# gunrock/mini

Measured on AMD Instinct MI355X. Metric: MTEPS (million traversed edges/sec) BFS advance+filter, RMAT-22, higher is better.
Workload: dtype int32

## Files before the change

### include/mgx/bfs_fused.hpp

```cpp
#pragma once
#include <cstdlib>
#include <cstring>

#include "runtime.hpp"
#include "env.hpp"
#include "wave.hpp"

namespace mgx {

constexpr int BFS_MAX_TRACE = 4096;
constexpr int BFS_VSHIFT = 38;
constexpr u64 BFS_EMASK = (1ull << BFS_VSHIFT) - 1ull;

struct bfs_ctrl_t {
  u64 cursor[3];
  u64 pad_a_[13];
  u64 lcursor[3];
  u64 pad_b_[13];
  u64 ledges[3];
  u64 pad_c_[13];
  u64 reached;
  u64 pad_d_[15];
  u64 merged_new;
  u64 sum_edges;
  u64 sum_frontier;
  u64 sum_long_edges;
  u64 sum_long_vertices;
  u64 claims;
  u64 claims_level[64];
  u64 pull_edges;
  int done;
  int levels;
  int pull;
  int push_levels;
  int d2_append_level;
// ... 173 lines not shown
  c->vshort_slots = 0;
  c->lazy_slot = -1;
  c->lazy_slots = 0;
  c->cold_slot = -1;
  c->cold_slots = 0;
  c->mini_slots = 0;
  for (int i = 0; i < 4; ++i) c->mini_blocks[i] = 0u;
  c->reached_mini = 0;
  c->d2_frozen_level = -1;
  for (int i = 0; i < 16; ++i) ((u32*)c->d2_level_kind)[i] = 0u;
  for (int i = 0; i < 64; ++i) c->d2_level_new[i] = 0u;
  c->sssp_thr = 0x7f7fffffu;
  c->sssp_far_cnt[0] = c->sssp_far_cnt[1] = 0;
  c->sssp_far_min[0] = c->sssp_far_min[1] = 0x7f7fffffu;
  for (int i = 0; i < 64; ++i) c->stamp[i] = 0;
}

__host__ __device__ __forceinline__ u32 bfs_lq_pad(u32 deg) { return (deg + 63u) & ~63u; }
__host__ __device__ __forceinline__ u32 bfs_lq_degree(u32 entry, u32 next_entry) {
  return ((next_entry & ~63u) - (entry & ~63u)) - ((64u - (entry & 63u)) & 63u);
}

__device__ __forceinline__ void bfs_seed_queue(const bfs_fused_args_t& a, u32 row) {
  bfs_ctrl_t* c = a.ctrl;
  const u32 ro = a.row_offsets[row];
  const u32 deg = a.row_offsets[row + 1] - ro;
  const bool is_long = a.long_min > 0 && deg >= (u32)a.long_min;
  (is_long ? a.lq_row : a.fr_row)[0][0] = ro;
  (is_long ? a.lq_off : a.fr_off)[0][0] = is_long ? (deg & 63u) : 0u;
  (is_long ? c->lcursor : c->cursor)[0] = deg ? ((1ull << BFS_VSHIFT) | (u64)(is_long ? bfs_lq_pad(deg) : deg)) : 0ull;
  if (is_long) c->ledges[0] = deg;
}

__global__ __launch_bounds__(BLOCK) void k_bfs_fused_init(bfs_fused_args_t a, int src, long long nwords, const bfs_ctrl_t* prev_ctrl,
                                                          bfs_ctrl_t* prev_head, int head_words) {
  if (prev_head && blockIdx.x == 0) {
    const u32* const from = (const u32*)prev_ctrl;
    u32* const to = (u32*)prev_head;
    for (int i = threadIdx.x; i < head_words; i += BLOCK) to[i] = from[i];
    __syncthreads();
  }
  const int src_old = src;
  if (a.new_of_old) src = a.new_of_old[src];
  const long long tid = (long long)blockIdx.x * BLOCK + threadIdx.x;
  const long long nth = (long long)gridDim.x * BLOCK;
  const long long n = a.n;
  for (long long i = tid; i < (n + 3) / 4; i += nth) {
    if (i * 4 + 4 <= n) {
      const long long j = i * 4;
      const int4 l = make_int4(src_old == j ? 0 : -1, src_old == j + 1 ? 0 : -1, src_old == j + 2 ? 0 : -1,
                               src_old == j + 3 ? 0 : -1);
      *(int4*)(a.labels + j) = l;
      *(u32*)(a.mark + i * 4) = 0u;
    } else {
      for (long long j = i * 4; j < n; ++j) { a.labels[j] = (j == src_old) ? 0 : -1; a.mark[j] = 0; }
    }
  }
  const u32 src_bit = 1u << (src & 31);
  for (long long w = tid; w < nwords; w += nth) {
    const u32 seed = (w == (src >> 5)) ? src_bit : 0u;
    a.visited[w] = seed;
    a.frontier_bits[w] = seed;
  }
  if (tid == 0) {
    bfs_ctrl_reset(a.ctrl);
    bfs_slot_marks_clear(a, 0);
    bfs_slot_marks_clear(a, 1);
    bfs_seed_queue(a, (u32)src);
  }
}

__device__ __forceinline__ bool bfs_open_level(const bfs_fused_args_t& a, int level, int slot) {
  bfs_ctrl_t* const c = a.ctrl;
  const u64 cur = c->cursor[slot % 3];
  const u64 lcur = c->lcursor[slot % 3];
  const long long nf = (long long)(cur >> BFS_VSHIFT) + (long long)(lcur >> BFS_VSHIFT);
  const u64 long_edges = c->ledges[slot % 3];
  const u64 E = (cur & BFS_EMASK) + long_edges;
  c->cursor[(slot + 2) % 3] = 0;
  c->lcursor[(slot + 2) % 3] = 0;
  c->ledges[(slot + 2) % 3] = 0;
  if (level < 64) c->stamp[level] = __builtin_amdgcn_s_memrealtime();
  if (nf == 0) {
    if (!c->done) { c->done = 1; c->levels = level; }
    return false;
  }
  if (level < BFS_MAX_TRACE) c->trace[level] = ((u64)nf << BFS_VSHIFT) | E;
  c->sum_edges += E;
  c->sum_frontier += (u64)nf;
  c->sum_long_edges += long_edges;
  c->sum_long_vertices += lcur >> BFS_VSHIFT;
  if (a.mode == 1 && !c->pull) {
    const float unvisited = (float)((long long)a.n - (long long)c->reached);
    if (unvisited < (float)nf * a.alpha) c->pull = 1;
  }
  if (!c->pull) c->push_levels += 1;
  return true;
}

__device__ __forceinline__ bool bfs_level_pulls(const bfs_fused_args_t& a, const bfs_ctrl_t* c, int slot) {
  if (a.mode != 1) return false;
  if (c->pull) return true;
// ... 542 lines not shown
  u32* __restrict__ const out_row_s = a.fr_row[(slot + 1) & 1];
  u32* __restrict__ const out_off_s = a.fr_off[(slot + 1) & 1];
  u32* __restrict__ const out_row_l = a.lq_row[(slot + 1) & 1];
  u32* __restrict__ const out_off_l = a.lq_off[(slot + 1) & 1];
  const u64 base_s = s_base[0], base_l = s_base[1];
#pragma unroll
  for (int q = 0; q < 16; ++q) {
    if ((new16 >> q) & 1u) {
      const u32 deg = ro[q + 1] - ro[q];
      if (deg >= long_min) {
        const u64 at = (base_l >> BFS_VSHIFT) + (ex_l >> 40);
        out_row_l[at] = ro[q];
        out_off_l[at] = (u32)((base_l & BFS_EMASK) + (ex_l & DEGMASK)) | (deg & 63u);
        ex_l += CNT1 | (u64)bfs_lq_pad(deg);
      } else if (deg) {
        const u64 at = (base_s >> BFS_VSHIFT) + (ex_s >> 40);
        out_row_s[at] = ro[q];
        out_off_s[at] = (u32)((base_s & BFS_EMASK) + (ex_s & DEGMASK));
        ex_s += CNT1 | (u64)deg;
      }
    }
  }
}

__global__ void k_bfs_publish(const bfs_ctrl_t* __restrict__ c, bfs_ctrl_t* __restrict__ host, u64* host_seq, u64 seq, int words) {
  const u32* const src = (const u32*)c;
  u32* const dst = (u32*)host;
  for (int i = threadIdx.x; i < words; i += blockDim.x) dst[i] = src[i];
  __threadfence_system();
  __syncthreads();
  if (threadIdx.x == 0) __hip_atomic_store(host_seq, seq, __ATOMIC_RELEASE, __HIP_MEMORY_SCOPE_SYSTEM);
}

struct bfs_run_opts_t {
  int cold_test = -1;
  int merged = 1;
  int dense = -1;
  int vshort = -1;
  long long chain = -1;
  int pack24 = 1;
  int hot_units = 1;
  int cold_pack = 1;
  int src_plan = 1;
  int defer_words = -1;
  int defer_mul = 1, defer_div = 1;
  int do_chain = 1;
  int merged_pull = 1;
  int seed_chain = 1;
  int tail_chain = 1;
  int tail_front = 1;
  int chain_big = -1;
  int cold = 1;
  int lazy = -1;
  long long defer = -1;
  int spin = -1;
  int build_list = 0;
  int mini = 1;
  int many_spare = 0;
#ifdef MGX_LAB
  int flags = 0;
  int build_diag = 0;
  int dense_diag = 0;
#endif
  static bfs_run_opts_t from_env() {
    bfs_run_opts_t o;
    auto geti = [](const char* name, int& out) { if (const char* e = mgx::env(name)) out = atoi(e); };
    auto getll = [](const char* name, long long& out) { if (const char* e = mgx::env(name)) out = atoll(e); };
    geti("MGX_BFS_COLD_TEST", o.cold_test);
    geti("MGX_BFS_MERGED_PUSH", o.merged);
    geti("MGX_BFS_DENSE", o.dense);
    geti("MGX_BFS_VSHORT", o.vshort);
    getll("MGX_BFS_CHAIN_MAX_EDGES", o.chain);
    geti("MGX_BFS_BUILD_LIST", o.build_list);
    getll("MGX_BFS_DEFER", o.defer);
    geti("MGX_BFS_DEFER_WORDS", o.defer_words);
    geti("MGX_BFS_SRC_PLAN", o.src_plan);
    geti("MGX_BFS_PACK24", o.pack24);
    geti("MGX_BFS_COLD_PACK", o.cold_pack);
    geti("MGX_BFS_HOT_UNITS", o.hot_units);
    geti("MGX_BFS_COLD", o.cold);
    if (const char* e = mgx::env("MGX_BFS_DEFER_REACH")) {
      o.defer_mul = atoi(e);
      const char* sl = strchr(e, '/');
      o.defer_div = sl ? atoi(sl + 1) : 1;
      if (o.defer_div < 1) o.defer_div = 1;
    }
    geti("MGX_BFS_SEED_CHAIN", o.seed_chain);
    geti("MGX_BFS_MERGED_PULL", o.merged_pull);
    geti("MGX_BFS_DO_CHAIN", o.do_chain);
    geti("MGX_BFS_TAIL_CHAIN", o.tail_chain);
    geti("MGX_BFS_TAIL_FRONT", o.tail_front);
    geti("MGX_BFS_CHAIN_BIG_EDGES", o.chain_big);
    geti("MGX_BFS_MINI", o.mini);
    if (o.many_spare < 0) o.many_spare = 0;
    geti("MGX_BFS_LAZY", o.lazy);
    if (o.lazy > (1 << 20)) o.lazy = 1 << 20;
#ifdef MGX_LAB
    geti("MGX_BFS_FLAGS", o.flags);
    geti("MGX_BFS_BUILD_DIAG", o.build_diag);
    geti("MGX_BFS_DENSE_DIAG", o.dense_diag);
#else
#endif
    return o;
  }
};

struct bfs_fused_state_t {
  bfs_run_opts_t opts = bfs_run_opts_t::from_env();
  mem_t<u32> visited;
  mem_t<unsigned char> mark;
  mem_t<u32> frontier_bits;
  mem_t<u32> fr_row[2];
  mem_t<u32> fr_off[2];
  mem_t<u32> lq_row[2];
  mem_t<u32> lq_off[2];
  mem_t<bfs_ctrl_t> ctrl;
  mem_t<u32> flush_buf;
  unsigned defer_min_marks = 2048;
  bfs_ctrl_t* host_ctrl = nullptr;
  u64* host_seq = nullptr;
  u64 seq = 0;
  bool spin = true;
  int n = 0;
  int levels_per_sync = 2;
  int slots_hint = 5;
  int slots_used = 0;
  bool time_batches = false;
  unsigned chain_max_edges = 4096;
  unsigned vshort_div = 8;
  unsigned chain_big_edges = 4096;
  int recent_need[4] = {1, 1, 1, 1}, recent_at = 0;
  int cls_max[3] = {0, 0, 0}, cls_at[3] = {0, 0, 0};
  int auto_spare = 0, clean_batches = 0;
  int tail_from = 1 << 30;
  unsigned lazy_div = 4;
  mem_t<u32> slot_marks;
  mem_t<u32> cold_flush;
  unsigned dense_div = 2;
  int long_min = LONG_MIN_DEFAULT;
  bool count_marks = false;
  int time_kernels = 0;
  unsigned hot_min_edges = 65536;
  hipEvent_t ev0 = nullptr, ev1 = nullptr;
  double level_kernel_ms = 0.0;
  long long level_kernel_launches = 0;
  float batch_ms[256];
  int batches = 0;
  static constexpr int EV_POOL = 96;
  hipEvent_t wev[EV_POOL] = {};
  double wave_kernel_ms = 0.0;
  long long wave_kernel_launches = 0;
  double stream_kernel_ms = 0.0;
  long long stream_kernel_launches = 0;
  float level_stream_ms[64] = {};
  float level_wave_ms[64] = {};

  bfs_fused_state_t(int num_nodes, standard_context_t& ctx) : n(num_nodes) {
    size_t words = (size_t)(num_nodes + 31) / 32 + 8;
    if (words < 65536) words = 65536;
    visited = mem_t<u32>(words, ctx);
    frontier_bits = mem_t<u32>(words, ctx);
    mark = mem_t<unsigned char>((size_t)num_nodes + 64, ctx);
    MGX_HIP(hipMemsetAsync(visited.data(), 0, words * sizeof(u32), ctx.stream()));
    MGX_HIP(hipMemsetAsync(frontier_bits.data(), 0, words * sizeof(u32), ctx.stream()));
    for (int i = 0; i < 2; ++i) {
      fr_row[i] = mem_t<u32>((size_t)num_nodes + 1, ctx);
      fr_off[i] = mem_t<u32>((size_t)num_nodes + 1, ctx);
      lq_row[i] = mem_t<u32>((size_t)num_nodes + 1, ctx);
      lq_off[i] = mem_t<u32>((size_t)num_nodes + 1, ctx);
    }
// ... 24 lines not shown
```

### include/mgx/bfs_fused_mini.hpp

```cpp
#pragma once
#include "bfs_fused.hpp"
#include "bfs_fused_chain.hpp"

namespace mgx {

constexpr int BFS_MINI_WGS = 64;
constexpr int BFS_MINI_LCAP = 4096;
constexpr int BFS_MINI_WCAP = 8192;
constexpr u32 BFS_MINI_EDGES_LATE = 131072;
constexpr u32 BFS_MINI_EDGES_EARLY = 32768;
constexpr u32 BFS_MINI_SHORT_ROWS = 65536;
constexpr size_t bfs_mini_lds_bytes() {
  return (size_t)(2 * BFS_MINI_LCAP + 4) * 4 + (size_t)BFS_MINI_WCAP * 4 + 64 * 8 + 256;
}

__device__ __forceinline__ bool bfs_level_is_mini(const bfs_fused_args_t& a, const bfs_ctrl_t* c, int slot) {
  if (a.mode != 0 || c->lazy_slot == slot) return false;
  const u64 cur = c->cursor[slot % 3], lcur = c->lcursor[slot % 3];
  const u64 E = (cur & BFS_EMASK) + c->ledges[slot % 3];
  const bool late = c->reached * 4ull >= (u64)(u32)a.n;
  return (lcur >> BFS_VSHIFT) <= (u64)BFS_MINI_LCAP && (cur >> BFS_VSHIFT) <= (u64)BFS_MINI_SHORT_ROWS &&
         E <= (u64)(late ? BFS_MINI_EDGES_LATE : BFS_MINI_EDGES_EARLY);
}

template <int NT>
__global__ __launch_bounds__(NT) void k_bfs_mini(bfs_fused_args_t a, int arg) {
  constexpr int NW = NT / WAVE;
  constexpr u64 CNT1 = 1ull << 40;
  constexpr u64 DEGMASK = CNT1 - 1ull;
  extern __shared__ __attribute__((aligned(16))) char smem[];
  u32* const s_loff = (u32*)smem;
  u32* const s_lrow = s_loff + BFS_MINI_LCAP + 4;
  u32* const s_win = s_lrow + BFS_MINI_LCAP;
  u64* const s_scan = (u64*)(s_win + BFS_MINI_WCAP);
  __shared__ int s_cnt, s_maxdeg;
  __shared__ u64 s_base[2];
  __shared__ u32 s_long_true;
  bfs_ctrl_t* const c = a.ctrl;
  int slot, level;
  bfs_resolve(c, arg, slot, level);
  if (c->done) return;
  const u64 cur = c->cursor[slot % 3], lcur = c->lcursor[slot % 3];
  const u64 ledges = c->ledges[slot % 3];
  const int nf_s = (int)(cur >> BFS_VSHIFT), nf_l = (int)(lcur >> BFS_VSHIFT);
  const u32 Es = (u32)(cur & BFS_EMASK), Rl = (u32)(lcur & BFS_EMASK);
  const int in = slot & 1, out = (slot + 1) & 1;
  const bool first_thread = blockIdx.x == 0 && threadIdx.x == 0;
  if (nf_s + nf_l == 0) {
    if (first_thread) {
      c->cursor[(slot + 2) % 3] = 0; c->lcursor[(slot + 2) % 3] = 0; c->ledges[(slot + 2) % 3] = 0;
      if (level < 64) c->stamp[level] = __builtin_amdgcn_s_memrealtime();
      if (!c->done) { c->done = 1; c->levels = level; }
    }
    return;
  }
  const long long gtid = (long long)blockIdx.x * NT + threadIdx.x, gthreads = (long long)gridDim.x * NT;
  if (!bfs_level_is_mini(a, c, slot)) {
    const bool lazy = c->lazy_slot == slot;
    const bool fb = c->fb_slot == slot;
    if (!lazy) {
      for (long long i = gtid; i < nf_s; i += gthreads) { a.fr_row[out][i] = a.fr_row[in][i]; a.fr_off[out][i] = a.fr_off[in][i]; }
      for (long long i = gtid; i < nf_l; i += gthreads) { a.lq_row[out][i] = a.lq_row[in][i]; a.lq_off[out][i] = a.lq_off[in][i]; }
    }
    __syncthreads();
    if (threadIdx.x == 0) {
      __threadfence();
      if (atomicAdd(&c->mini_blocks[slot & 3], 1u) == gridDim.x - 1u) {
        c->mini_blocks[slot & 3] = 0u;
        c->cursor[(slot + 1) % 3] = cur; c->lcursor[(slot + 1) % 3] = lcur; c->ledges[(slot + 1) % 3] = ledges;
        c->cursor[(slot + 2) % 3] = 0; c->lcursor[(slot + 2) % 3] = 0; c->ledges[(slot + 2) % 3] = 0;
        c->slot_level[(slot + 1) & 3] = level;
        c->flush_count[(slot + 1) & 1] = 0;
        bfs_slot_marks_clear(a, slot + 1);
        if (lazy) c->lazy_slot = slot + 1;
        if (fb) c->fb_slot = slot + 1;
      }
    }
    return;
  }
  if (first_thread) {
    const u64 E = (u64)Es + ledges;
    c->cursor[(slot + 2) % 3] = 0; c->lcursor[(slot + 2) % 3] = 0; c->ledges[(slot + 2) % 3] = 0;
    if (level < 64) c->stamp[level] = __builtin_amdgcn_s_memrealtime();
    if (level < BFS_MAX_TRACE) c->trace[level] = ((u64)(nf_s + nf_l) << BFS_VSHIFT) | E;
    c->sum_edges += E;
    c->sum_frontier += (u64)(nf_s + nf_l);
    c->sum_long_edges += ledges;
    c->sum_long_vertices += (u64)nf_l;
    c->push_levels += 1;
    c->small_levels += 1;
    c->mini_slots += 1;
    c->slots += 1;
    c->slot_level[(slot + 1) & 3] = level + 1;
    c->flush_count[(slot + 1) & 1] = 0;
    bfs_slot_marks_clear(a, slot + 1);
    c->fb_slot = -1;
  }
  const int lane = lane_id();
  const int wave = threadIdx.x / WAVE;
  const u32 long_min = a.long_min > 0 ? (u32)a.long_min : 0xFFFFFFFFu;
// ... 38 lines not shown
        if (tot_l >> 40) atomicAdd(&c->ledges[(slot + 1) % 3], (u64)s_long_true);
      }
      __syncthreads();
      if (deg) {
        const u64 b = is_long ? s_base[1] : s_base[0];
        const u64 at = is_long ? ex_l : ex_s;
        const u64 pos = (b >> BFS_VSHIFT) + (at >> 40);
        (is_long ? out_row_l : out_row_s)[pos] = ro;
        (is_long ? out_off_l : out_off_s)[pos] = (u32)((b & BFS_EMASK) + (at & DEGMASK)) | (is_long ? (deg & 63u) : 0u);
      }
      __syncthreads();
    }
    if (threadIdx.x == 0) s_cnt = 0;
    __syncthreads();
  };
  auto visit = [&](bool act, u32 d) {
    bool win = false;
    if (act) {
      const u32 bit = 1u << (d & 31u);
      const u32 seen = a.visited[d >> 5];
      if (!(seen & bit)) win = !(atomicOr(a.visited + (d >> 5), bit) & bit);
    }
    const u64 bal = __ballot(win);
    if (bal) {
      int at = 0;
      if (lane == 0) at = atomicAdd(&s_cnt, __popcll(bal));
      at = __builtin_amdgcn_readfirstlane(at);
      if (win) { s_win[at + rank_in_mask(bal)] = d; ++found; }
    }
  };

  {
    const u32 U = Rl >> 6;
    const u32 Wt = (u32)gridDim.x * NW, w0 = (u32)blockIdx.x * NW + (u32)wave;
    const u32 iters = (U + Wt - 1u) / Wt;
    for (u32 t = 0; t < iters; ++t) {
      const u32 u = w0 + t * Wt;
      bool act = false;
      u32 d = 0;
      if (u < U) {
        const u32 r0 = u << 6;
        int lo = 0, hi = nf_l;
        while (hi - lo > 1) { const int mid = (lo + hi) >> 1; if ((s_loff[mid] & ~63u) <= r0) lo = mid; else hi = mid; }
        const u32 e0 = s_loff[lo];
        const u32 deg = bfs_lq_degree(e0, s_loff[lo + 1]);
        const u32 rank = r0 - (e0 & ~63u) + (u32)lane;
        act = rank < deg;
        if (act) d = (u32)a.col_indices[s_lrow[lo] + rank];
      }
      visit(act, d);
      __syncthreads();
      const int cnt_now = s_cnt;
      __syncthreads();
      if (cnt_now > BFS_MINI_WCAP - NT) flush();
    }
  }
  if (nf_s > 0 && (u64)Es >= 4ull * (u64)nf_s) {
    const u32* __restrict__ fr_row = a.fr_row[in];
    const u32* __restrict__ fr_off = a.fr_off[in];
    const u32 iters = (Es + (u32)gthreads - 1u) / (u32)gthreads;
    for (u32 t = 0; t < iters; ++t) {
      const u64 r64 = (u64)gtid + (u64)t * (u64)gthreads;
      const bool act = r64 < (u64)Es;
      const u32 r = act ? (u32)r64 : 0u;
      int lo = 0, hi = nf_s;
      while (hi - lo > 1) { const int mid = (lo + hi) >> 1; if (fr_off[mid] <= r) lo = mid; else hi = mid; }
      const u32 d = act ? (u32)a.col_indices[fr_row[lo] + (r - fr_off[lo])] : 0u;
// ... 10 lines not shown
    const u32 iters = ((u32)nf_s + (u32)gthreads - 1u) / (u32)gthreads;
    for (u32 t = 0; t < iters; ++t) {
      const long long i = gtid + (long long)t * gthreads;
      u32 row = 0, deg = 0;
      if (i < nf_s) {
        const u32 e0 = fr_off[i], e1 = (i + 1 < nf_s) ? fr_off[i + 1] : Es;
        row = fr_row[i];
        deg = e1 - e0;
      }
      int wmax = (int)deg;
#pragma unroll
      for (int sh = WAVE / 2; sh > 0; sh >>= 1) { const int o = __shfl_xor(wmax, sh, WAVE); wmax = o > wmax ? o : wmax; }
      if (lane == 0 && wmax) atomicMax(&s_maxdeg, wmax);
      __syncthreads();
      const u32 kmax = (u32)s_maxdeg;
      for (u32 k = 0; k < kmax; ++k) {
        const bool act = k < deg;
        const u32 d = act ? (u32)a.col_indices[row + k] : 0u;
        visit(act, d);
        __syncthreads();
        const int cnt_now = s_cnt;
        __syncthreads();
        if (cnt_now > BFS_MINI_WCAP - NT) flush();
      }
      __syncthreads();
      if (threadIdx.x == 0) s_maxdeg = 0;
      __syncthreads();
    }
  }
  flush();
  found = (int)wave_sum((u32)found);
  if (lane == 0 && found) atomicAdd(&c->reached_mini, (u64)found);
}

}
```

### include/mgx/bfs_fused_run.hpp

```cpp
#pragma once
#include <cstring>
#include <vector>
#include <unistd.h>
#include "bfs_fused.hpp"
#include "bfs_fused_chain.hpp"
#include "bfs_fused_cold.hpp"
#include "bfs_fused_dense.hpp"
#include "bfs_fused_mini.hpp"
#include "bfs_fused_pull.hpp"
#include "bfs_fused_stream.hpp"
#include "bfs_fused_vshort.hpp"
#include "bfs_fused_sparse.hpp"
#include "bfs_fused_wave.hpp"
#include "row_layout.hpp"

namespace mgx {

struct bfs_layout_t {
  const int* row_offsets = nullptr;
  const int* col_indices = nullptr;
  const int* new_of_old = nullptr;
  const int* old_of_new = nullptr;
  const row_layout_t* rows = nullptr;
  const unsigned* src_shapes = nullptr;
  int src_shapes_long_min = 0;
};
static_assert(row_layout_t::MAX_SLICES == BFS_COLD_MAX_SLICES, "row_layout_t's slice tables hold this many slices");

constexpr int BFS_SRC_UNKNOWN = 0, BFS_SRC_ABSORB = 1, BFS_SRC_SKIP = 2;

constexpr int BFS_STREAM_HOTW2 = 20400;
constexpr int BFS_WAVE_HOTW = 18000;
constexpr int BFS_DENSE_HOTW = BFS_STREAM_HOTW2 - 16;
// ... 59 lines not shown
    if ((PART == 0 || PART == 1) && blockIdx.x == 0) bfs_chain_body<1024>(a, p.slot, p.level);
    return;
  }
  if ((PART == 0 || PART == 1) && blockIdx.x == 0 && threadIdx.x == 0) bfs_slot_open(a, p);
  if (p.empty || PART == 1) return;
  if (p.pulls) {
    if (a.merged_pull && PART != 3) {
      extern __shared__ __attribute__((aligned(16))) char smem_pull[];
      bfs_pull_body<1024>(a, blockIdx.x, gridDim.x, (unsigned long long*)smem_pull);
    }
    return;
  }
  const u32 ncold = (!COLDT && a.cold_dst && (PART == 0 || PART == 2)) ? a.cold_wgs[a.cold_slices] : 0u;
  if (blockIdx.x < ncold) {
    if (p.cold || p.colds) bfs_cold_body<1024>(a, p.slot, blockIdx.x, p.level, p.cold, p.colds);
    return;
  }
  if (a.cold_all && p.cold) return;
  const u32 blk = blockIdx.x - ncold, nblk = gridDim.x - ncold;
  const bool long_part = PART == 2 || (PART == 0 && blk < nstream);
  if (long_part) {
    const u32 bi = blk;
    if (!COLDT && p.dense) bfs_dense_body<1024, BFS_DENSE_HOTW>(a, p.slot, bi, nstream, p.level, p.cold);
    else bfs_stream_body<1024, BFS_STREAM_HOTW2, 8, COLDT, false, true>(a, p.slot, bi, nstream, p.level);
  } else {
    const u32 first = PART == 0 ? nstream : 0u;
    const u32 bi = blk - first;
    const u32 nb = nblk - first;
    if (!COLDT && p.vshort) bfs_vshort_body<1024, BFS_DENSE_HOTW>(a, p.slot, bi, nb, p.level, p.colds);
    else bfs_wave_body<1024, BFS_WAVE_HOTW, COLDT, false>(a, p.slot, bi, nb, p.level);
  }
}

__global__ __launch_bounds__(1024) void k_bfs_chain_inplace(bfs_fused_args_t a, int arg) {
  const bfs_ctrl_t* const c = a.ctrl;
  int slot, level;
  bfs_resolve(c, arg, slot, level);
  const u64 cur = c->cursor[slot % 3], lcur = c->lcursor[slot % 3];
  if (c->done || ((cur | lcur) >> BFS_VSHIFT) == 0) return;
  if (c->lazy_slot == slot) return;
  if (!bfs_level_is_chained(a, cur, lcur, c->ledges[slot % 3], a.chain_big_edges, BFS_CHAIN_CAP_BIG)) return;
  bfs_chain_body<1024, true, BFS_CHAIN_CAP_BIG>(a, slot, level);
}

#ifdef MGX_LAB
__global__ __launch_bounds__(1024, 8) void k_bfs_push_stream_diag(bfs_fused_args_t a, int arg) {
  const bfs_slot_plan_t p = bfs_slot_plan(a, arg);
  if (p.empty || p.chained) return;
  bfs_stream_body<1024, BFS_STREAM_HOTW2, 8, false, true, true>(a, p.slot, blockIdx.x, gridDim.x, p.level);
}
#endif

template <bool COLDT>
__global__ __launch_bounds__(1024, 8) void k_bfs_push_level(bfs_fused_args_t a, int level, u32 nstream, int open_here, u32 ncold) {
  if (bfs_d2_frozen(a.ctrl, level)) return;
  const int skip = open_here >> 4;
  open_here &= 15;
  const bool appends = bfs_d2_level_appends(a, level);
  if (open_here && blockIdx.x == gridDim.x - 1 && threadIdx.x == 0) {
    bfs_begin_level(a, level, open_here == 2);
    bfs_slot_marks_clear(a, level + 1);
    a.ctrl->flush_count[(level + 1) & 1] = 0;
    a.ctrl->d2_append_level = appends ? level : -1;
  }
  if (appends) {
    if (!(skip & 1)) bfs_d2_sparse_body<1024>(a, level, blockIdx.x, gridDim.x);
    return;
  }
  const bool dense = bfs_long_is_dense(a, a.ctrl, level, a.ctrl->lcursor[level % 3]) && (!COLDT || a.cold_dst != nullptr);
  const bool cold = dense && a.cold_dst != nullptr;
  if (blockIdx.x < ncold) {
    if (cold && !(skip & 1)) {
      if (blockIdx.x == 0 && threadIdx.x == 0) { a.ctrl->cold_slot = level; a.ctrl->cold_slots += 1; }
      bfs_cold_body<1024>(a, level, blockIdx.x, level, true, false);
    }
    return;
  }
  const u32 blk = blockIdx.x - ncold, nblk = gridDim.x - ncold;
  if (blk < nstream ? (skip & 2) != 0 : (skip & 4) != 0) return;
  if (blk < nstream) {
    if (dense) {
      if (blk == 0 && threadIdx.x == 0) a.ctrl->dense_slots += 1;
      bfs_dense_body<1024, BFS_DENSE_HOTW>(a, level, blk, nstream, level, cold);
    } else bfs_stream_body<1024, BFS_STREAM_HOTW2, 8, COLDT, false, true>(a, level, blk, nstream, level);
  } else if (a.d2_front && bfs_short_is_dense(a, a.ctrl, level, a.ctrl->cursor[level % 3])) {
    if (blk == nstream && threadIdx.x == 0) a.ctrl->vshort_slots += 1;
    bfs_vshort_body<1024, BFS_DENSE_HOTW, COLDT>(a, level, blk - nstream, nblk - nstream, level);
  } else bfs_wave_body<1024, BFS_WAVE_HOTW, COLDT, false>(a, level, blk - nstream, nblk - nstream, level);
}

inline void bfs_set_kernel_attributes() {
  static unsigned char seen[64] = {};
  device_once_t once(seen);
  if (!once) return;
#define MGX_SET_LDS(K_) MGX_HIP(hipFuncSetAttribute((const void*)K_, hipFuncAttributeMaxDynamicSharedMemorySize, 160 * 1024))
  MGX_SET_LDS((k_bfs_push<false, 0>)); MGX_SET_LDS((k_bfs_push<true, 0>));
  MGX_SET_LDS((k_bfs_push<false, 1>)); MGX_SET_LDS((k_bfs_push<true, 1>));
  MGX_SET_LDS((k_bfs_push<false, 2>)); MGX_SET_LDS((k_bfs_push<true, 2>));
  MGX_SET_LDS((k_bfs_push<false, 3>)); MGX_SET_LDS((k_bfs_push<true, 3>));
#ifdef MGX_LAB
  MGX_SET_LDS(k_bfs_push_stream_diag);
#endif
  MGX_SET_LDS(k_bfs_chain_inplace);
  MGX_HIP(hipFuncSetAttribute((const void*)k_bfs_mini<1024>, hipFuncAttributeMaxDynamicSharedMemorySize, (int)bfs_mini_lds_bytes()));
  MGX_SET_LDS(k_bfs_push_level<false>);
  MGX_SET_LDS(k_bfs_push_level<true>);
#undef MGX_SET_LDS
}

inline bool bfs_cold_test(int n, int forced) {
  if (forced >= 0) return forced != 0;
  return (long long)n >= 8ll * 32 * BFS_STREAM_HOTW;
}

template <int PART>
inline void bfs_launch_push_part(const bfs_fused_args_t& a, int arg, standard_context_t& ctx, bool coldt, unsigned grid, u32 nstream) {
  if (coldt) hipLaunchKernelGGL((k_bfs_push<true, PART>), dim3(grid), dim3(1024), bfs_push_lds_bytes(), ctx.stream(), a, arg, nstream);
  else hipLaunchKernelGGL((k_bfs_push<false, PART>), dim3(grid), dim3(1024), bfs_push_lds_bytes(), ctx.stream(), a, arg, nstream);
}

inline void bfs_launch_push(const bfs_fused_args_t& a, int level, standard_context_t& ctx, int open_here, bool coldt, u32 grid_div = 1) {
  if (grid_div < 1u) grid_div = 1u;
  u32 per = (u32)ctx.num_cus * 2 / grid_div;
  if (per < 32u) per = 32u;
  const u32 nstream = a.long_min > 0 ? per : 0u;
  const u32 nwave = per;
  const u32 ncold = a.cold_dst ? a.cold_wgs[a.cold_slices] : 0u;
  if (coldt) hipLaunchKernelGGL(k_bfs_push_level<true>, dim3(ncold + nstream + nwave), dim3(1024), bfs_push_lds_bytes(), ctx.stream(), a, level, nstream, open_here, ncold);
  else hipLaunchKernelGGL(k_bfs_push_level<false>, dim3(ncold + nstream + nwave), dim3(1024), bfs_push_lds_bytes(), ctx.stream(), a, level, nstream, open_here, ncold);
}

struct bfs_launch_plan_t {
  bfs_fused_args_t a;
  bool coldt = false, build2_ok = false;
  bool minis = false;
  u32 nstream = 0, nwave = 0, ncold = 0;
// ... 149 lines not shown
  if (deg > chain_cap) {
    const bool is_long = a.long_min > 0 && deg >= (u64)a.long_min;
    E = deg; rs = is_long ? 0 : 1; rl = is_long ? 1 : 0;
  } else if (e1 > chain_cap) {
    E = e1; rs = s1; rl = l1;
  } else {
    return BFS_SRC_UNKNOWN;
  }
  const bool mini = rl <= (u64)BFS_MINI_LCAP && rs <= (u64)BFS_MINI_SHORT_ROWS && E <= (u64)BFS_MINI_EDGES_EARLY;
  return mini ? BFS_SRC_ABSORB : BFS_SRC_SKIP;
}
inline int bfs_class_slots(const bfs_fused_state_t& st, int cls) {
  if (cls == BFS_SRC_UNKNOWN) return st.slots_hint;
  if (st.cls_at[cls] > 0) return st.cls_max[cls];
  if (cls == BFS_SRC_SKIP && st.cls_at[BFS_SRC_ABSORB] > 0) return st.cls_max[BFS_SRC_ABSORB] + 1 > st.slots_hint ? st.cls_max[BFS_SRC_ABSORB] + 1 : st.slots_hint;
  return st.slots_hint;
}

inline void bfs_enqueue_chain_inplace(const bfs_launch_plan_t& plan, int slot, hipStream_t s) {
  hipLaunchKernelGGL(k_bfs_chain_inplace, dim3(1), dim3(1024), bfs_chain_lds_bytes(BFS_CHAIN_CAP_BIG), s, plan.a, bfs_slot_arg(slot));
}
inline void bfs_enqueue_mini(const bfs_launch_plan_t& plan, int slot, hipStream_t s) {
  hipLaunchKernelGGL(k_bfs_mini<1024>, dim3(BFS_MINI_WGS), dim3(1024), bfs_mini_lds_bytes(), s, plan.a, bfs_slot_arg(slot));
}
inline int bfs_enqueue_start(const bfs_fused_state_t& st, const bfs_launch_plan_t& plan, int src, standard_context_t& ctx,
                             const bfs_ctrl_t* prev_ctrl = nullptr, bfs_ctrl_t* prev_head = nullptr, int head_words = 0,
                             bool front_mini = true) {
  hipStream_t s = ctx.stream();
  hipLaunchKernelGGL(k_bfs_fused_init, dim3(grid_for(((long long)st.n + 3) / 4, BLOCK, ctx.num_cus * 8)), dim3(BLOCK), 0, s, plan.a, src,
                     plan.nwords, prev_ctrl, prev_head, head_words);
  if (plan.a.chain_big_edges) bfs_enqueue_chain_inplace(plan, 0, s);
  if (plan.minis && front_mini) { bfs_enqueue_mini(plan, 0, s); return 1; }
  return 0;
}
inline void bfs_enqueue_build(const bfs_fused_state_t& st, const bfs_launch_plan_t& plan, int arg, hipStream_t s) {
  if (st.opts.build_list || !plan.build2_ok)
    hipLaunchKernelGGL((k_bfs_build<512, true>), dim3(bfs_build_grid(st.n, 512)), dim3(512), 0, s, plan.a, arg,
                       (const u32*)nullptr, plan.labels, st.n, 1, 0, 1);
  else
    hipLaunchKernelGGL(k_bfs_build2<512>, dim3(bfs_build_grid(st.n, 512)), dim3(512), 0, s, plan.a, arg, plan.labels, st.n);
}
inline void bfs_enqueue_slot(const bfs_fused_state_t& st, const bfs_launch_plan_t& plan, int slot, standard_context_t& ctx) {
  hipStream_t s = ctx.stream();
  const int arg = bfs_slot_arg(slot);
  if (plan.a.chain_big_edges && slot > 0 && slot >= st.tail_from && st.opts.tail_chain && st.opts.tail_front && !plan.minis)
    bfs_enqueue_chain_inplace(plan, slot, s);
  bfs_launch_push_part<0>(plan.a, arg, ctx, plan.coldt, plan.nstream + plan.ncold + plan.nwave, plan.nstream);
  if (plan.mode == 1 && !plan.a.merged_pull)
    hipLaunchKernelGGL(k_bfs_pull_level<256>, dim3(ctx.num_cus * 8), dim3(256), 0, s, plan.a, arg);
  bfs_enqueue_build(st, plan, arg, s);
}

inline void bfs_learn_slots(bfs_fused_state_t& st, const bfs_fused_args_t& a, const bfs_ctrl_t* hc, int mode, int trace_avail, bool minis = false,
                            int cls = BFS_SRC_UNKNOWN) {
  st.slots_hint = hc->slots > 0 ? hc->slots : 1;
  st.tail_from = 1 << 30;
  if (!(a.chain_big_edges && st.opts.tail_chain)) return;
  const int lv = hc->levels < trace_avail ? hc->levels : trace_avail;
  int kind[64];
  const int L = lv < 64 ? lv : 64;
  bool pulled = false;
  u64 reached = 1;
  int extra_big = lv > 64 ? lv - 64 : 0;
  (void)extra_big;
  for (int l = 0; l < L; ++l) {
    const u64 t = hc->trace[l];
// ... 163 lines not shown
    MGX_HIP(hipStreamSynchronize(s));
  }
  bfs_learn_slots(st, a, st.host_ctrl, mode, BFS_MAX_TRACE, plan.minis, cls);
}

constexpr size_t bfs_head_bytes() { return offsetof(bfs_ctrl_t, trace) + 64 * sizeof(u64); }
constexpr size_t bfs_many_head_bytes() { return (bfs_head_bytes() + 63) & ~(size_t)63; }
inline bfs_ctrl_t* bfs_many_head(char* heads, int i) { return (bfs_ctrl_t*)(heads + (size_t)i * bfs_many_head_bytes()); }

inline int bfs_fused_run_many(bfs_fused_state_t& st, const int* row_offsets, const int* col_indices, int* labels,
                              const int* srcs, int count, standard_context_t& ctx, char* heads, const bfs_layout_t* layout = nullptr,
                              int mode = 0, float alpha = 0.f, const int* in_offsets = nullptr, const int* in_indices = nullptr) {
  if (count <= 0) return 0;
  hipStream_t s = ctx.stream();
  auto run_one = [&](int i) {
    bfs_layout_t one;
    if (layout) { one = *layout; if (one.src_shapes) one.src_shapes += (size_t)i * 4; }
    bfs_fused_run(st, row_offsets, col_indices, labels, srcs[i], ctx, layout ? &one : nullptr, mode, alpha, in_offsets, in_indices);
  };
  const bfs_launch_plan_t plan = bfs_fused_plan(st, row_offsets, col_indices, labels, ctx, layout, mode, alpha, in_offsets, in_indices);
  const bfs_fused_args_t& a = plan.a;
  constexpr int head_words = (int)(bfs_head_bytes() / 4);
  bool uneven = false;
  for (int i = 1; i < 4 && i < st.recent_at; ++i) uneven |= st.recent_need[i] != st.recent_need[0];
  int nslots = st.slots_hint + st.opts.many_spare + (mode == 1 ? (uneven ? 2 : 1) : 0) + st.auto_spare;
  if (nslots > 30) {
    for (int i = 0; i < count; ++i) {
      run_one(i);
      memcpy(bfs_many_head(heads, i), st.host_ctrl, bfs_head_bytes());
    }
    return 0;
  }
  if (nslots < 1) nslots = 1;
  const int saved_tail = st.tail_from;
  st.tail_from = plan.minis ? (1 << 30) : nslots - 1;
  const bool tail = a.chain_big_edges && st.opts.tail_chain;
  std::vector<int> last_slots((size_t)count, nslots), classes((size_t)count, BFS_SRC_UNKNOWN);
  bfs_launch_plan_t plan_tail = plan;
  plan_tail.a.chain_big_edges = BFS_CHAIN_CAP_BIG;
  for (int i = 0; i < count; ++i) {
    const int cls = bfs_classify_source(st, plan, layout, srcs[i], i);
    int my_slots = cls == BFS_SRC_UNKNOWN ? nslots : bfs_class_slots(st, cls) + st.opts.many_spare + st.auto_spare;
    if (my_slots > 30) my_slots = 30;
    if (my_slots < 1) my_slots = 1;
    int sl = bfs_enqueue_start(st, plan, srcs[i], ctx, i > 0 ? st.ctrl.data() : (const bfs_ctrl_t*)nullptr,
                               i > 0 ? bfs_many_head(heads, i - 1) : (bfs_ctrl_t*)nullptr, head_words, cls != BFS_SRC_SKIP);
    for (int k = 0; k < my_slots; ++k, ++sl) bfs_enqueue_slot(st, plan, sl, ctx);
    if (plan.minis) { bfs_enqueue_mini(plan, sl, s); ++sl; }
    if (tail) bfs_enqueue_chain_inplace(plan_tail, sl, s);
    last_slots[(size_t)i] = sl;
    classes[(size_t)i] = cls;
  }
  st.tail_from = saved_tail;
  const u64 seq = ++st.seq;
  hipLaunchKernelGGL(k_bfs_publish, dim3(1), dim3(256), 0, s, (const bfs_ctrl_t*)st.ctrl.data(), bfs_many_head(heads, count - 1), st.host_seq, seq, head_words);
  MGX_CHECK_LAUNCH("fused BFS (batch of sources): kernel launch");
  {
    volatile u64* const flag = st.host_seq;
    long long spins = 0;
    while (*flag != seq) {
      if (++spins > 20000000LL) { MGX_HIP(hipStreamSynchronize(s)); break; }
      __builtin_ia32_pause();
    }
    __atomic_thread_fence(__ATOMIC_ACQUIRE);
  }
  int reruns = 0;
  bool redo_last = false;
  for (int i = 0; i < count; ++i) {
    bfs_ctrl_t* const h = bfs_many_head(heads, i);
    const int last_slot = last_slots[(size_t)i];
    if (!h->done) {
      const u64 next = h->cursor[last_slot % 3] | h->lcursor[last_slot % 3];
      if ((next >> BFS_VSHIFT) == 0) { h->done = 1; h->levels = h->slot_level[last_slot & 3]; }
    }
    if (h->done) { bfs_learn_slots(st, a, h, mode, 64, plan.minis, classes[(size_t)i]); continue; }
    run_one(i);
    memcpy(h, st.host_ctrl, bfs_head_bytes());
    ++reruns;
    if (i != count - 1) redo_last = true;
  }
  if (redo_last) run_one(count - 1);
  st.slots_used = last_slots[(size_t)count - 1];
  if (reruns > 0) { if (st.auto_spare < 4) ++st.auto_spare; st.clean_batches = 0; }
  else if (st.auto_spare > 0 && ++st.clean_batches >= 8) { --st.auto_spare; st.clean_batches = 0; }
  return reruns;
}

}
// ... 1 lines not shown
```

### include/mgx/env.hpp

```cpp
#pragma once
#include <cstdio>
#include <cstdlib>
#include <cstring>

namespace mgx {

struct env_switch_t { const char* name; const char* what; };

inline const env_switch_t* env_switches(int* count) {
  static const env_switch_t table[] = {
    {"MGX_BFS_DENSE", "0 / N: unit-block body for long rows off / a level takes it from frontier edges >= units / N"},
    {"MGX_BFS_VSHORT", "0 / N: short rows vertex by vertex off / threshold divisor"},
    {"MGX_BFS_LAZY", "0 / N: lazy queues off / the build writes no queues behind a push that stored >= n / N marks"},
    {"MGX_BFS_COLD", "0 / 2 (lab: 1): cold-edge pass off / on"},
    {"MGX_BFS_COLD_LISTS", "0 / 1 (lab: 2): whether the layout builds the long rows' cold-edge lists"},
    {"MGX_BFS_COLD_PACK", "0: keep the 8-byte cold pairs instead of the packed 4-byte ones"},
    {"MGX_BFS_COLD_TEST", "0 / 1: bitmap probe of cold neighbours off / on (default: by graph size)"},
    {"MGX_BFS_FLAT_LISTS", "0: a flat graph keeps the ordinary layout instead of all-entry pair lists"},
    {"MGX_BFS_HOT_UNITS", "0: no second copy of the unit blocks without the cold lists' entries"},
    {"MGX_BFS_PACK24", "0: 32-bit unit-block entries instead of the 24-bit copy"},
    {"MGX_BFS_MINI", "0 / 2: no M launches / M launches on every graph (default: from 2^22 vertices on)"},
    {"MGX_BFS_SEED_CHAIN", "0: the chain of small levels at the start runs inside slot 0's push launch"},
    {"MGX_BFS_TAIL_CHAIN", "0: no in-place chain launch behind the last slots"},
    {"MGX_BFS_TAIL_FRONT", "0: no chain in front of the last slots"},
    {"MGX_BFS_CHAIN_BIG_EDGES", "largest level an in-place chain launch runs (edges)"},
    {"MGX_BFS_CHAIN_MAX_EDGES", "largest level block 0 runs inside the push launch (0: no chains)"},
    {"MGX_BFS_MERGED_PUSH", "0: the parts of a slot's push as separate launches"},
    {"MGX_BFS_MERGED_PULL", "0: direction-optimising runs: the bottom-up sweep as a launch of its own"},
    {"MGX_BFS_DO_CHAIN", "0: direction-optimising runs: no chains of small top-down levels"},
    {"MGX_BFS_DEFER", "0 / N: deferred hot marks off / a workgroup flushes its bitmap above N claims"},
    {"MGX_BFS_DEFER_REACH", "\"mul/div\": a level defers its hot marks while reached * mul < range * div"},
    {"MGX_BFS_DEFER_WORDS", "words of the bitmap prefix whose marks are deferred (default: all)"},
    {"MGX_BFS_BUILD_LIST", "1: the list-based queue build of round 1"},
    {"MGX_BFS_SRC_PLAN", "0: no per-source launch plan"},
    {"MGX_BFS_LONG_MIN", "long-row threshold of the layout (entries)"},
    {"MGX_BFS_HOT_MIN_EDGES", "smallest level that copies the bitmap prefix to LDS (edges)"},
    {"MGX_BFS_FLAGS", "(lab) instrumented stream kernel; results wrong by design"},
    {"MGX_BFS_BUILD_DIAG", "(lab) parts of the queue build switched off; results wrong by design"},
    {"MGX_BFS_DENSE_DIAG", "(lab) parts of the unit-block body switched off; results wrong by design"},
    {"MGX_SSSP_DENSE", "0 / N: no sweep for heavy iterations / an iteration is heavy from m / N frontier edges"},
    {"MGX_SSSP_HOT_MIN_EDGES", "smallest iteration that keeps the hubs' distance bounds in LDS (edges)"},
    {"MGX_SSSP_BUILD_LIST", "1: list-based queue build"},
    {"MGX_NR_SLICED", "0: the unit blocks instead of the long rows by slice of their destinations"},
    {"MGX_NR_SLICES", "number of hot slices (default: by graph size; at most what the id range holds)"},
    {"MGX_NR_FOLD_DEGS", "\"a/b/c\": the fold's tiers (a workgroup / a wave / eight lanes per row) from these degrees"},
    {"MGX_NR_SUBSET", "0: subset frontiers take the general kernel"},
    {"MGX_NR_PARTS", "1 / 2 / 3: timing runs of the short rows only / the long rows only / both"},
    {"MGX_DIST_SPEC", "0: a host look per level instead of the level plan"},
    {"MGX_DIST_SPARSE_PUSH", "0: every level sweeps the marks"},
    {"MGX_DIST_DECLARE_MUL", "a sweep fills its id list unless the push stored > N x capacity marks (0: always)"},
    {"MGX_DIST_FUSED_MERGE", "0: OR-merge and queue build as two launches"},
    {"MGX_DIST_BUILD_LIST", "1: list-based queue build on the ranks"},
    {"MGX_DIST_PUSH_SPLIT", "1: the parts of a rank's push as separate launches (statistics)"},
    {"MGX_DIST_DEFER", "0: no deferred hot marks on the ranks"},
// ... 27 lines not shown
```

Before: 449,300.

## Overlap consecutive BFS sources in a batch using a second traversal state

Adds a second pooled traversal state so consecutive sources in a batch alternate between two sets of buffers. At each seam between sources, the previous source's tail mini/chain launches are merged into a single launch with the next source's init (and its first chain), which cuts serialized small launches and idle time between traversals. The final publish copies both control heads. In exchange it allocates a second full set of frontier and bitmap buffers and adds more complex slot bookkeeping across sources.

```diff
diff --git a/include/mgx/bfs_fused.hpp b/include/mgx/bfs_fused.hpp
--- a/include/mgx/bfs_fused.hpp
+++ b/include/mgx/bfs_fused.hpp
@@ -1,6 +1,7 @@
 #pragma once
 #include <cstdlib>
 #include <cstring>
+#include <memory>
 
 #include "runtime.hpp"
 #include "env.hpp"
@@ -240,18 +241,19 @@
   if (is_long) c->ledges[0] = deg;
 }
 
-__global__ __launch_bounds__(BLOCK) void k_bfs_fused_init(bfs_fused_args_t a, int src, long long nwords, const bfs_ctrl_t* prev_ctrl,
-                                                          bfs_ctrl_t* prev_head, int head_words) {
-  if (prev_head && blockIdx.x == 0) {
+template <int NT>
+__device__ __forceinline__ void bfs_init_body(const bfs_fused_args_t& a, int src, long long nwords, const bfs_ctrl_t* prev_ctrl,
+                                              bfs_ctrl_t* prev_head, int head_words, u32 blk, u32 nblk) {
+  if (prev_head && blk == 0) {
     const u32* const from = (const u32*)prev_ctrl;
     u32* const to = (u32*)prev_head;
-    for (int i = threadIdx.x; i < head_words; i += BLOCK) to[i] = from[i];
+    for (int i = threadIdx.x; i < head_words; i += NT) to[i] = from[i];
     __syncthreads();
   }
   const int src_old = src;
   if (a.new_of_old) src = a.new_of_old[src];
-  const long long tid = (long long)blockIdx.x * BLOCK + threadIdx.x;
-  const long long nth = (long long)gridDim.x * BLOCK;
+  const long long tid = (long long)blk * NT + threadIdx.x;
+  const long long nth = (long long)nblk * NT;
   const long long n = a.n;
   for (long long i = tid; i < (n + 3) / 4; i += nth) {
     if (i * 4 + 4 <= n) {
@@ -276,6 +278,10 @@
     bfs_slot_marks_clear(a, 1);
     bfs_seed_queue(a, (u32)src);
   }
+}
+__global__ __launch_bounds__(BLOCK) void k_bfs_fused_init(bfs_fused_args_t a, int src, long long nwords, const bfs_ctrl_t* prev_ctrl,
+                                                          bfs_ctrl_t* prev_head, int head_words) {
+  bfs_init_body<BLOCK>(a, src, nwords, prev_ctrl, prev_head, head_words, blockIdx.x, gridDim.x);
 }
 
 __device__ __forceinline__ bool bfs_open_level(const bfs_fused_args_t& a, int level, int slot) {
@@ -884,6 +890,17 @@
   if (threadIdx.x == 0) __hip_atomic_store(host_seq, seq, __ATOMIC_RELEASE, __HIP_MEMORY_SCOPE_SYSTEM);
 }
 
+__global__ void k_bfs_publish2(const bfs_ctrl_t* __restrict__ c0, bfs_ctrl_t* __restrict__ host0, const bfs_ctrl_t* __restrict__ c1,
+                               bfs_ctrl_t* __restrict__ host1, u64* host_seq, u64 seq, int words) {
+  for (int i = threadIdx.x; i < words; i += blockDim.x) {
+    ((u32*)host0)[i] = ((const u32*)c0)[i];
+    ((u32*)host1)[i] = ((const u32*)c1)[i];
+  }
+  __threadfence_system();
+  __syncthreads();
+  if (threadIdx.x == 0) __hip_atomic_store(host_seq, seq, __ATOMIC_RELEASE, __HIP_MEMORY_SCOPE_SYSTEM);
+}
+
 struct bfs_run_opts_t {
   int cold_test = -1;
   int merged = 1;
@@ -908,6 +925,7 @@
   int spin = -1;
   int build_list = 0;
   int mini = 1;
+  int batch_overlap = 1;
   int many_spare = 0;
 #ifdef MGX_LAB
   int flags = 0;
@@ -944,6 +962,7 @@
     geti("MGX_BFS_TAIL_FRONT", o.tail_front);
     geti("MGX_BFS_CHAIN_BIG_EDGES", o.chain_big);
     geti("MGX_BFS_MINI", o.mini);
+    geti("MGX_BFS_BATCH_OVERLAP", o.batch_overlap);
     if (o.many_spare < 0) o.many_spare = 0;
     geti("MGX_BFS_LAZY", o.lazy);
     if (o.lazy > (1 << 20)) o.lazy = 1 << 20;
@@ -954,6 +973,37 @@
 #else
 #endif
     return o;
+  }
+};
+
+struct bfs_alt_state_t {
+  mem_t<char> pool;
+  u32 *visited = nullptr, *frontier_bits = nullptr;
+  unsigned char* mark = nullptr;
+  u32 *fr_row[2] = {}, *fr_off[2] = {}, *lq_row[2] = {}, *lq_off[2] = {};
+  bfs_ctrl_t* ctrl = nullptr;
+  u32* slot_marks = nullptr;
+  int* labels = nullptr;
+  static std::unique_ptr<bfs_alt_state_t> make(int num_nodes, size_t words, standard_context_t& ctx) {
+    std::unique_ptr<bfs_alt_state_t> t(new bfs_alt_state_t());
+    const size_t n = (size_t)num_nodes;
+    size_t at = 0;
+    auto take = [&](size_t bytes) { const size_t off = at; at += (bytes + 255) & ~(size_t)255; return off; };
+    const size_t o_vis = take(words * 4), o_fb = take(words * 4), o_mark = take(n + 64), o_ctrl = take(sizeof(bfs_ctrl_t)),
+                 o_sm = take((size_t)2 * BFS_MARK_CTRS * BFS_MARK_STRIDE * 4), o_lab = take((n + 4) * 4);
+    size_t o_q[8];
+    for (int i = 0; i < 8; ++i) o_q[i] = take((n + 1) * 4);
+    char* b = nullptr;
+    if (hipMalloc((void**)&b, at) != hipSuccess || !b) { (void)hipGetLastError(); return nullptr; }
+    t->pool = mem_t<char>::adopt(b, at);
+    t->visited = (u32*)(b + o_vis); t->frontier_bits = (u32*)(b + o_fb); t->mark = (unsigned char*)(b + o_mark);
+    t->ctrl = (bfs_ctrl_t*)(b + o_ctrl); t->slot_marks = (u32*)(b + o_sm); t->labels = (int*)(b + o_lab);
+    for (int i = 0; i < 2; ++i) {
+      t->fr_row[i] = (u32*)(b + o_q[i]); t->fr_off[i] = (u32*)(b + o_q[2 + i]);
+      t->lq_row[i] = (u32*)(b + o_q[4 + i]); t->lq_off[i] = (u32*)(b + o_q[6 + i]);
+    }
+    MGX_HIP(hipMemsetAsync(t->visited, 0, o_mark - o_vis, ctx.stream()));
+    return t;
   }
 };
 
@@ -988,6 +1038,8 @@
   unsigned lazy_div = 4;
   mem_t<u32> slot_marks;
   mem_t<u32> cold_flush;
+  std::unique_ptr<bfs_alt_state_t> alt;
+  bool alt_refused = false;
   unsigned dense_div = 2;
   int long_min = LONG_MIN_DEFAULT;
   bool count_marks = false;
diff --git a/include/mgx/bfs_fused_mini.hpp b/include/mgx/bfs_fused_mini.hpp
--- a/include/mgx/bfs_fused_mini.hpp
+++ b/include/mgx/bfs_fused_mini.hpp
@@ -24,7 +24,7 @@
 }
 
 template <int NT>
-__global__ __launch_bounds__(NT) void k_bfs_mini(bfs_fused_args_t a, int arg) {
+__device__ __forceinline__ void bfs_mini_body(const bfs_fused_args_t& a, int arg, u32 blk, u32 nblk) {
   constexpr int NW = NT / WAVE;
   constexpr u64 CNT1 = 1ull << 40;
   constexpr u64 DEGMASK = CNT1 - 1ull;
@@ -45,7 +45,7 @@
   const int nf_s = (int)(cur >> BFS_VSHIFT), nf_l = (int)(lcur >> BFS_VSHIFT);
   const u32 Es = (u32)(cur & BFS_EMASK), Rl = (u32)(lcur & BFS_EMASK);
   const int in = slot & 1, out = (slot + 1) & 1;
-  const bool first_thread = blockIdx.x == 0 && threadIdx.x == 0;
+  const bool first_thread = blk == 0 && threadIdx.x == 0;
   if (nf_s + nf_l == 0) {
     if (first_thread) {
       c->cursor[(slot + 2) % 3] = 0; c->lcursor[(slot + 2) % 3] = 0; c->ledges[(slot + 2) % 3] = 0;
@@ -54,7 +54,7 @@
     }
     return;
   }
-  const long long gtid = (long long)blockIdx.x * NT + threadIdx.x, gthreads = (long long)gridDim.x * NT;
+  const long long gtid = (long long)blk * NT + threadIdx.x, gthreads = (long long)nblk * NT;
   if (!bfs_level_is_mini(a, c, slot)) {
     const bool lazy = c->lazy_slot == slot;
     const bool fb = c->fb_slot == slot;
@@ -65,7 +65,7 @@
     __syncthreads();
     if (threadIdx.x == 0) {
       __threadfence();
-      if (atomicAdd(&c->mini_blocks[slot & 3], 1u) == gridDim.x - 1u) {
+      if (atomicAdd(&c->mini_blocks[slot & 3], 1u) == nblk - 1u) {
         c->mini_blocks[slot & 3] = 0u;
         c->cursor[(slot + 1) % 3] = cur; c->lcursor[(slot + 1) % 3] = lcur; c->ledges[(slot + 1) % 3] = ledges;
         c->cursor[(slot + 2) % 3] = 0; c->lcursor[(slot + 2) % 3] = 0; c->ledges[(slot + 2) % 3] = 0;
@@ -170,7 +170,7 @@
 
   {
     const u32 U = Rl >> 6;
-    const u32 Wt = (u32)gridDim.x * NW, w0 = (u32)blockIdx.x * NW + (u32)wave;
+    const u32 Wt = nblk * NW, w0 = blk * NW + (u32)wave;
     const u32 iters = (U + Wt - 1u) / Wt;
     for (u32 t = 0; t < iters; ++t) {
       const u32 u = w0 + t * Wt;
@@ -247,5 +247,9 @@
   found = (int)wave_sum((u32)found);
   if (lane == 0 && found) atomicAdd(&c->reached_mini, (u64)found);
 }
-
-}
+template <int NT>
+__global__ __launch_bounds__(NT) void k_bfs_mini(bfs_fused_args_t a, int arg) {
+  bfs_mini_body<NT>(a, arg, blockIdx.x, gridDim.x);
+}
+
+}
diff --git a/include/mgx/bfs_fused_run.hpp b/include/mgx/bfs_fused_run.hpp
--- a/include/mgx/bfs_fused_run.hpp
+++ b/include/mgx/bfs_fused_run.hpp
@@ -1,4 +1,5 @@
 #pragma once
+#include <cassert>
 #include <cstring>
 #include <vector>
 #include <unistd.h>
@@ -124,7 +125,7 @@
   }
 }
 
-__global__ __launch_bounds__(1024) void k_bfs_chain_inplace(bfs_fused_args_t a, int arg) {
+__device__ __forceinline__ void bfs_chain_inplace_body(const bfs_fused_args_t& a, int arg) {
   const bfs_ctrl_t* const c = a.ctrl;
   int slot, level;
   bfs_resolve(c, arg, slot, level);
@@ -133,6 +134,30 @@
   if (c->lazy_slot == slot) return;
   if (!bfs_level_is_chained(a, cur, lcur, c->ledges[slot % 3], a.chain_big_edges, BFS_CHAIN_CAP_BIG)) return;
   bfs_chain_body<1024, true, BFS_CHAIN_CAP_BIG>(a, slot, level);
+}
+__global__ __launch_bounds__(1024) void k_bfs_chain_inplace(bfs_fused_args_t a, int arg) {
+  bfs_chain_inplace_body(a, arg);
+}
+
+struct bfs_seam_init_t {
+  long long nwords;
+  const bfs_ctrl_t* prev_ctrl;
+  bfs_ctrl_t* prev_head;
+  int src, head_words;
+};
+static_assert(2 * sizeof(bfs_fused_args_t) + sizeof(bfs_seam_init_t) + 64 <= 4096, "a seam launch's two argument structs fit the 4 KB of kernel arguments");
+__global__ __launch_bounds__(1024) void k_bfs_seam_mini_init(bfs_fused_args_t a, int arg_a, bfs_fused_args_t b, bfs_seam_init_t init) {
+  if (blockIdx.x < (u32)BFS_MINI_WGS) bfs_mini_body<1024>(a, arg_a, blockIdx.x, (u32)BFS_MINI_WGS);
+  else bfs_init_body<1024>(b, init.src, init.nwords, init.prev_ctrl, init.prev_head, init.head_words, blockIdx.x - (u32)BFS_MINI_WGS,
+                           gridDim.x - (u32)BFS_MINI_WGS);
+}
+__global__ __launch_bounds__(1024) void k_bfs_seam_chain_chain(bfs_fused_args_t a, int arg_a, bfs_fused_args_t b, int arg_b) {
+  if (blockIdx.x == 0) bfs_chain_inplace_body(a, arg_a);
+  else bfs_chain_inplace_body(b, arg_b);
+}
+__global__ __launch_bounds__(1024) void k_bfs_seam_chain_init(bfs_fused_args_t a, int arg_a, bfs_fused_args_t b, bfs_seam_init_t init) {
+  if (blockIdx.x == 0) bfs_chain_inplace_body(a, arg_a);
+  else bfs_init_body<1024>(b, init.src, init.nwords, init.prev_ctrl, init.prev_head, init.head_words, blockIdx.x - 1u, gridDim.x - 1u);
 }
 
 #ifdef MGX_LAB
@@ -194,6 +219,9 @@
   MGX_SET_LDS(k_bfs_push_stream_diag);
 #endif
   MGX_SET_LDS(k_bfs_chain_inplace);
+  MGX_SET_LDS(k_bfs_seam_chain_chain);
+  MGX_SET_LDS(k_bfs_seam_chain_init);
+  MGX_HIP(hipFuncSetAttribute((const void*)k_bfs_seam_mini_init, hipFuncAttributeMaxDynamicSharedMemorySize, (int)bfs_mini_lds_bytes()));
   MGX_HIP(hipFuncSetAttribute((const void*)k_bfs_mini<1024>, hipFuncAttributeMaxDynamicSharedMemorySize, (int)bfs_mini_lds_bytes()));
   MGX_SET_LDS(k_bfs_push_level<false>);
   MGX_SET_LDS(k_bfs_push_level<true>);
@@ -409,6 +437,54 @@
   if (plan.a.chain_big_edges) bfs_enqueue_chain_inplace(plan, 0, s);
   if (plan.minis && front_mini) { bfs_enqueue_mini(plan, 0, s); return 1; }
   return 0;
+}
+inline bool bfs_fused_plan_alt(bfs_fused_state_t& st, const bfs_launch_plan_t& plan, standard_context_t& ctx, bfs_launch_plan_t& p) {
+  if (!st.alt && !st.alt_refused) {
+    st.alt = bfs_alt_state_t::make(st.n, st.bitmap_words(), ctx);
+    st.alt_refused = !st.alt;
+  }
+  if (!st.alt) return false;
+  bfs_alt_state_t& t = *st.alt;
+  p = plan;
+  bfs_fused_args_t& a = p.a;
+  a.labels = p.labels = t.labels;
+  a.visited = t.visited;
+  a.mark = t.mark;
+  a.frontier_bits = t.frontier_bits;
+  for (int i = 0; i < 2; ++i) {
+    a.fr_row[i] = t.fr_row[i]; a.fr_off[i] = t.fr_off[i];
+    a.lq_row[i] = t.lq_row[i]; a.lq_off[i] = t.lq_off[i];
+  }
+  a.ctrl = t.ctrl;
+  a.slot_marks = t.slot_marks;
+  return true;
+}
+inline void bfs_enqueue_seam(const bfs_fused_state_t& st, const bfs_launch_plan_t& plan_a, const bfs_launch_plan_t& tail_a, int sl_a,
+                             const bfs_launch_plan_t& plan_b, int src, bfs_ctrl_t* prev_head, int head_words, standard_context_t& ctx) {
+  hipStream_t s = ctx.stream();
+  bfs_seam_init_t init;
+  init.nwords = plan_b.nwords;
+  init.prev_ctrl = plan_b.a.ctrl;
+  init.prev_head = prev_head;
+  init.src = src;
+  init.head_words = head_words;
+  const int want = grid_for(((long long)st.n + 3) / 4, 1024, 1 << 20);
+  if (plan_a.minis) {
+    int ninit = ctx.num_cus - BFS_MINI_WGS;
+    if (ninit < 64) ninit = 64;
+    if (ninit > want) ninit = want;
+    hipLaunchKernelGGL(k_bfs_seam_mini_init, dim3(BFS_MINI_WGS + ninit), dim3(1024), bfs_mini_lds_bytes(), s, plan_a.a, bfs_slot_arg(sl_a),
+                       plan_b.a, init);
+    hipLaunchKernelGGL(k_bfs_seam_chain_chain, dim3(2), dim3(1024), bfs_chain_lds_bytes(BFS_CHAIN_CAP_BIG), s, tail_a.a, bfs_slot_arg(sl_a + 1),
+                       plan_b.a, bfs_slot_arg(0));
+  } else {
+    int ninit = ctx.num_cus - 1;
+    if (ninit < 16) ninit = 16;
+    if (ninit > want) ninit = want;
+    hipLaunchKernelGGL(k_bfs_seam_chain_init, dim3(1 + ninit), dim3(1024), bfs_chain_lds_bytes(BFS_CHAIN_CAP_BIG), s, tail_a.a, bfs_slot_arg(sl_a),
+                       plan_b.a, init);
+    bfs_enqueue_chain_inplace(plan_b, 0, s);
+  }
 }
 inline void bfs_enqueue_build(const bfs_fused_state_t& st, const bfs_launch_plan_t& plan, int arg, hipStream_t s) {
   if (st.opts.build_list || !plan.build2_ok)
@@ -638,28 +714,59 @@
     return 0;
   }
   if (nslots < 1) nslots = 1;
-  const int saved_tail = st.tail_from;
+  struct tail_guard_t {
+    int& at; const int saved; bool armed;
+    void release() { if (armed) { at = saved; armed = false; } }
+    ~tail_guard_t() { release(); }
+  } tail_guard{st.tail_from, st.tail_from, true};
   st.tail_from = plan.minis ? (1 << 30) : nslots - 1;
   const bool tail = a.chain_big_edges && st.opts.tail_chain;
   std::vector<int> last_slots((size_t)count, nslots), classes((size_t)count, BFS_SRC_UNKNOWN);
-  bfs_launch_plan_t plan_tail = plan;
-  plan_tail.a.chain_big_edges = BFS_CHAIN_CAP_BIG;
+  bool overlap = st.opts.batch_overlap != 0 && mode == 0 && count >= 2 && tail && !st.alt_refused;
+  const int lead = (overlap && !st.alt) ? (count - 1 < 2 ? count - 1 : 2) : 0;
+  bfs_launch_plan_t plans[2] = {plan, plan}, tails[2];
+  for (int k = 0; k < 2; ++k) { tails[k] = plans[k]; tails[k].a.chain_big_edges = BFS_CHAIN_CAP_BIG; }
+  auto second_state = [&]() {
+    if (!bfs_fused_plan_alt(st, plan, ctx, plans[1])) { overlap = false; return; }
+    tails[1] = plans[1]; tails[1].a.chain_big_edges = BFS_CHAIN_CAP_BIG;
+  };
+  if (overlap && st.alt) second_state();
+  auto state_of = [&](int i) { return (overlap && i >= lead) ? ((count - 1 - i) & 1) : 0; };
+  int pending[2] = {-1, -1};
   for (int i = 0; i < count; ++i) {
     const int cls = bfs_classify_source(st, plan, layout, srcs[i], i);
     int my_slots = cls == BFS_SRC_UNKNOWN ? nslots : bfs_class_slots(st, cls) + st.opts.many_spare + st.auto_spare;
     if (my_slots > 30) my_slots = 30;
     if (my_slots < 1) my_slots = 1;
-    int sl = bfs_enqueue_start(st, plan, srcs[i], ctx, i > 0 ? st.ctrl.data() : (const bfs_ctrl_t*)nullptr,
-                               i > 0 ? bfs_many_head(heads, i - 1) : (bfs_ctrl_t*)nullptr, head_words, cls != BFS_SRC_SKIP);
-    for (int k = 0; k < my_slots; ++k, ++sl) bfs_enqueue_slot(st, plan, sl, ctx);
-    if (plan.minis) { bfs_enqueue_mini(plan, sl, s); ++sl; }
-    if (tail) bfs_enqueue_chain_inplace(plan_tail, sl, s);
+    const int me = state_of(i);
+    const bfs_launch_plan_t& P = plans[me];
+    bfs_ctrl_t* const prev_head = pending[me] >= 0 ? bfs_many_head(heads, pending[me]) : (bfs_ctrl_t*)nullptr;
+    pending[me] = i;
+    int sl;
+    if (i == 0 || state_of(i - 1) == me) {
+      sl = bfs_enqueue_start(st, P, srcs[i], ctx, prev_head ? P.a.ctrl : (const bfs_ctrl_t*)nullptr, prev_head, head_words, cls != BFS_SRC_SKIP);
+    } else {
+      const int sl_a = plan.minis ? last_slots[(size_t)i - 1] - 1 : last_slots[(size_t)i - 1];
+      bfs_enqueue_seam(st, plans[me ^ 1], tails[me ^ 1], sl_a, P, srcs[i], prev_head, head_words, ctx);
+      sl = 0;
+      if (plan.minis && cls != BFS_SRC_SKIP) { bfs_enqueue_mini(P, 0, s); sl = 1; }
+    }
+    for (int k = 0; k < my_slots; ++k, ++sl) bfs_enqueue_slot(st, P, sl, ctx);
+    if (overlap && i + 1 == lead && !st.alt) second_state();
+    const bool seam_behind = i + 1 < count && state_of(i + 1) != me;
+    if (plan.minis) { if (!seam_behind) bfs_enqueue_mini(P, sl, s); ++sl; }
+    if (tail && !seam_behind) bfs_enqueue_chain_inplace(tails[me], sl, s);
     last_slots[(size_t)i] = sl;
     classes[(size_t)i] = cls;
   }
-  st.tail_from = saved_tail;
+  tail_guard.release();
   const u64 seq = ++st.seq;
-  hipLaunchKernelGGL(k_bfs_publish, dim3(1), dim3(256), 0, s, (const bfs_ctrl_t*)st.ctrl.data(), bfs_many_head(heads, count - 1), st.host_seq, seq, head_words);
+  assert(pending[0] == count - 1);
+  if (pending[1] >= 0)
+    hipLaunchKernelGGL(k_bfs_publish2, dim3(1), dim3(256), 0, s, (const bfs_ctrl_t*)plans[0].a.ctrl, bfs_many_head(heads, pending[0]),
+                       (const bfs_ctrl_t*)plans[1].a.ctrl, bfs_many_head(heads, pending[1]), st.host_seq, seq, head_words);
+  else
+    hipLaunchKernelGGL(k_bfs_publish, dim3(1), dim3(256), 0, s, (const bfs_ctrl_t*)st.ctrl.data(), bfs_many_head(heads, count - 1), st.host_seq, seq, head_words);
   MGX_CHECK_LAUNCH("fused BFS (batch of sources): kernel launch");
   {
     volatile u64* const flag = st.host_seq;
diff --git a/include/mgx/env.hpp b/include/mgx/env.hpp
--- a/include/mgx/env.hpp
+++ b/include/mgx/env.hpp
@@ -20,6 +20,7 @@
     {"MGX_BFS_HOT_UNITS", "0: no second copy of the unit blocks without the cold lists' entries"},
     {"MGX_BFS_PACK24", "0: 32-bit unit-block entries instead of the 24-bit copy"},
     {"MGX_BFS_MINI", "0 / 2: no M launches / M launches on every graph (default: from 2^22 vertices on)"},
+    {"MGX_BFS_BATCH_OVERLAP", "0: a batch of sources runs in one traversal state, no launch shared by two traversals"},
     {"MGX_BFS_SEED_CHAIN", "0: the chain of small levels at the start runs inside slot 0's push launch"},
     {"MGX_BFS_TAIL_CHAIN", "0: no in-place chain launch behind the last slots"},
     {"MGX_BFS_TAIL_FRONT", "0: no chain in front of the last slots"},
```

New measurement: 461,800 (median of 6 runs). 1.03x the previous value.
